# flxrcz/hommx

Hardware: AMD Instinct MI355X
Metric: micro-cell solves/sec (higher is better)
Workload: dtype f64

## Files before the change

### hommx_amd/csrc/fused2d.hip

```cpp
#include <hip/hip_runtime.h>
#include <stdint.h>

#include <type_traits>

#include "kernels.h"
#include "sweep_acc.h"

#ifndef HOMMX_FUSED_WAVES_PER_SIMD
#define HOMMX_FUSED_WAVES_PER_SIMD 2
#endif

namespace hommx {

typedef double d4 __attribute__((ext_vector_type(4)));
typedef double d2 __attribute__((ext_vector_type(2)));

__device__ __forceinline__ double uniform_f64(double v) {
  return __hiloint2double(__builtin_amdgcn_readfirstlane(__double2hiint(v)),
                          __builtin_amdgcn_readfirstlane(__double2loint(v)));
}

struct CoefRow {
  double a0, a1;
  double a0m, a1m;
};

constexpr int MATP = 48;

template <int NB>
struct alignas(16) Lds {
  double mat[(NB + 1) * MATP];
  double ubuf[4 * NB];
  double tsc[16 * 17];
  double rrow[2][NB];
  double vrow[2][NB];
  double vnat[2][NB];
  double e0row[NB];
  double e1row[NB];
  double e0nat[NB];
  double e1nat[NB];
  double dgnat[NB];
  double cenat[NB + 2];
};
template <int NB>
struct alignas(16) LdsIso {
  static constexpr int PARK = NB == 32 ? 12 * 64 : 0;
  double ubuf[4 * NB];
  double tsc[16 * 17];
  double rrow[2][NB];
  double vrow[2][NB];
  double vnat[2][NB];
  double e0row[NB];
  double e0nat[NB];
  double dgnat[NB];
  double cenat[NB + 2];
  double park[PARK ? PARK : 1];
};

struct NoFact {};
template <int NB, bool FACT, bool ISO>
__global__ __launch_bounds__(64, (NB == 32 && ISO) ? 3 : HOMMX_FUSED_WAVES_PER_SIMD) void k_poisson2d_fused(
    const double* __restrict__ coef, const double* __restrict__ Mmat, double* __restrict__ out,
    int32_t* __restrict__ info, int n, long long ncells, const CoefSource src, std::conditional_t<FACT, double*, NoFact> fact
#ifdef HOMMX_FUSED_DEBUG
    , double* __restrict__ dbg
#endif
) {
  constexpr int NT = NB / 16, KK = NB / 4, CG = 64 / NB;
  constexpr int P = MATP;
  constexpr bool PARK = ISO && NB == 32;
  static_assert(!(FACT && ISO), "the factor record keeps the general path");
  __shared__ std::conditional_t<ISO, LdsIso<NB>, Lds<NB>> L;

  const long long cell = blockIdx.x;
  if (cell >= ncells) return;
  __builtin_assume(n >= 3);
  __builtin_assume(n <= NB);
  const int l = threadIdx.x;
  const int j = l & 15, k = l >> 4;
  const int c = l % NB, g = l / NB;
  const int lb = l - c;
  const int p0 = NB - n;
  const bool valid = c >= p0;
  const int cn = c - p0;
  const int cm = valid ? (c == p0 ? NB - 1 : c - 1) : c;
  const int cp = valid ? (c == NB - 1 ? p0 : c + 1) : c;
  const int prow = (c & 3) * KK + (c >> 2);

  const int ownB = (k + 1) * P + j;
  [[maybe_unused]] int leftB[NT];
#pragma unroll
  for (int tj = 0; tj < NT; ++tj) {
    const int col = 16 * tj + j;
    leftB[tj] = (k + 1) * P + (col == p0 ? NB - 1 : col - 1);
  }
#define OWN(ti, tj, r) (ownB + (16 * (ti) + 4 * (r)) * P + 16 * (tj))
#define LEFT(ti, tj, r) (leftB[tj] + (16 * (ti) + 4 * (r)) * P)
  [[maybe_unused]] unsigned matOff = 0;
  if constexpr (!ISO) matOff = accl::lds_offset(&L.mat[0]);
  [[maybe_unused]] const unsigned haloA = matOff + 8u * (unsigned)(p0 * P + j);

  const int mode = src.mode;
  const unsigned char* mask = static_cast<const unsigned char*>(src.table);
  const double* table = static_cast<const double*>(src.table);
  const double* cc = mode == COEF_STREAM ? coef + cell * (2ll * n * n) : coef + cell * 2;
  constexpr int NL = NB * NB / 64;
  double2 pv[NL];
  if (mode == COEF_STREAM) {
#pragma unroll
    for (int i = 0; i < NL; ++i) {
      const int el = 2 * l + 128 * i;
      pv[i] = el < 2 * n * n ? *reinterpret_cast<const double2*>(cc + el) : double2{0.0, 0.0};
    }
  }

  if constexpr (!ISO)
    for (int i = l; i < (NB + 1) * P; i += 64) L.mat[i] = 0.0;
  if (l == 0) L.cenat[0] = 0.0;

  double m00 = 1.0, m01 = 0.0, m10 = 0.0, m11 = 1.0;
  if (!ISO && Mmat) {
    const double* mp = Mmat + cell * 4;
    m00 = mp[0]; m01 = mp[1]; m10 = mp[2]; m11 = mp[3];
  }
  const double al = ISO ? 0.5 : uniform_f64(0.5 * (m00 * m00 + m10 * m10));
  const double be = ISO ? 0.5 : uniform_f64(0.5 * (m01 * m01 + m11 * m11));
  const double ga = ISO ? 0.0 : uniform_f64(0.5 * (m00 * m01 + m10 * m11));
  const double ab = ISO ? 1.0 : uniform_f64(al - 2.0 * ga + be);

  double ph0 = 0.0, ph1 = 0.0;
  if (mode != COEF_STREAM) {
    ph0 = cc[0];
    ph1 = cc[1];
  }
  const int nq = src.nq;
  auto sample = [&](long long el) {
    double acc = 0.0;
    for (int q = 0; q < nq; ++q)
      acc = add_rn(acc, mul_rn(src.weights[q], div_rn(1.0, add_rn(ph0, mul_rn(ph1, table[el * nq + q])))));
    return acc;
  };
  auto load_pair = [&](long long el, double& a0, double& a1) {
    if (mode == COEF_TWO_PHASE) {
      const uchar2 mk = *reinterpret_cast<const uchar2*>(mask + el);
      a0 = mk.x ? ph1 : ph0;
      a1 = mk.y ? ph1 : ph0;
    } else if (mode == COEF_AFFINE) {
      const double2 g2 = *reinterpret_cast<const double2*>(table + el);
      a0 = add_rn(ph0, mul_rn(ph1, g2.x));
      a1 = add_rn(ph0, mul_rn(ph1, g2.y));
    } else if (mode == COEF_RECIPROCAL) {
      a0 = sample(el);
      a1 = sample(el + 1);
    } else {
      const double2 v = *reinterpret_cast<const double2*>(cc + el);
      a0 = v.x; a1 = v.y;
    }
  };
  int esh;
  {
    int ef = 0;
    if (mode == COEF_STREAM) {
      int hm = 0;
#pragma unroll
      for (int i = 0; i < NL; ++i) hm = max(hm, max(__double2hiint(pv[i].x) & 0x7fffffff, __double2hiint(pv[i].y) & 0x7fffffff));
      ef = hm >> 20;
    } else {
      for (long long el = 2 * l; el < 2ll * n * n; el += 128) {
        double a0, a1;
        load_pair(el, a0, a1);
        const int f0 = (__double2hiint(a0) >> 20) & 0x7ff, f1 = (__double2hiint(a1) >> 20) & 0x7ff;
        ef = max(ef, max(f0, f1));
      }
    }
#pragma unroll
    for (int off = 32; off >= 1; off >>= 1) ef = max(ef, __shfl_xor(ef, off, 64));
    const int fm = (__double2hiint(6.0 * (al + be)) >> 20) & 0x7ff;
    const int sh = (ef == 0 || ef == 0x7ff ? 0 : ef - 1023) + (fm == 0 || fm == 0x7ff ? 0 : fm - 1023) + 2;
    esh = __builtin_amdgcn_readfirstlane(ef == 0 || ef == 0x7ff ? 0 : sh);
  }
  auto load_row = [&](int jc) {
    CoefRow r;
    r.a0 = 0.0; r.a1 = 0.0;
    if (valid) {
      load_pair(2 * (jc * n + cn), r.a0, r.a1);
      r.a0 = ldexp(r.a0, -esh);
      r.a1 = ldexp(r.a1, -esh);
    }
    r.a0m = __shfl(r.a0, lb + cm, 64);
    r.a1m = __shfl(r.a1, lb + cm, 64);
    return r;
  };
  auto st_diag = [&](const CoefRow& cur, const CoefRow& prev) {
    return valid ? cur.a0 * al + cur.a1 * be + cur.a0m * ab + prev.a0m * be + prev.a1m * al + prev.a1 * ab : 1.0;
  };
  auto st_E = [&](const CoefRow& cur, const CoefRow& prev) { return (cur.a0 + prev.a1) * (ga - al); };
  auto st_N = [&](const CoefRow& cur) { return (cur.a1 + cur.a0m) * (ga - be); };
  auto st_NE = [&](const CoefRow& cur) { return -ga * (cur.a0 + cur.a1); };
  auto st_p0 = [&](const CoefRow& cur, const CoefRow& prev) { return cur.a0 - cur.a0m - prev.a1m + prev.a1; };
  auto st_p1 = [&](const CoefRow& cur, const CoefRow& prev) { return cur.a1 + cur.a0m - prev.a0m - prev.a1; };

  [[maybe_unused]] auto band_write = [&](double dv, double ov, bool sym, bool clear) {
    if constexpr (!ISO) {
      if (g == 0) {
        const double d_ = clear ? 0.0 : dv, o_ = clear ? 0.0 : ov;
        L.mat[(c + 1) * P + c] = d_;
        if (valid) {
          L.mat[(cp + 1) * P + c] = o_;
          if (sym) L.mat[(c + 1) * P + cp] = o_;
        }
      }
    }
  };
  auto sub_band = [&](double (&x)[NT][NT][4], const double (&dgq)[NT], const double (&ceq)[NT], const double (&cemq)[NT]) {
#pragma unroll
    for (int t = 0; t < NT; ++t) {
      using namespace accl;
#define DIAG_LO(r) (OneLane<0, 4 * (r)>::lo | OneLane<1, 4 * (r) + 1>::lo | OneLane<2, 4 * (r) + 2>::lo | OneLane<3, 4 * (r) + 3>::lo)
#define DIAG_HI(r) (OneLane<0, 4 * (r)>::hi | OneLane<1, 4 * (r) + 1>::hi | OneLane<2, 4 * (r) + 2>::hi | OneLane<3, 4 * (r) + 3>::hi)
      masked_sub4<DIAG_LO(0), DIAG_HI(0), DIAG_LO(1), DIAG_HI(1), DIAG_LO(2), DIAG_HI(2), DIAG_LO(3), DIAG_HI(3)>(
          x[t][t][0], x[t][t][1], x[t][t][2], x[t][t][3], dgq[t]);
#define SUB_LO(r) (((r) ? OneLane<0, (4 * (r) - 1) & 15>::lo : 0u) | OneLane<1, 4 * (r)>::lo | OneLane<2, 4 * (r) + 1>::lo | OneLane<3, 4 * (r) + 2>::lo)
#define SUB_HI(r) (((r) ? OneLane<0, (4 * (r) - 1) & 15>::hi : 0u) | OneLane<1, 4 * (r)>::hi | OneLane<2, 4 * (r) + 1>::hi | OneLane<3, 4 * (r) + 2>::hi)
      masked_sub4<SUB_LO(0), SUB_HI(0), SUB_LO(1), SUB_HI(1), SUB_LO(2), SUB_HI(2), SUB_LO(3), SUB_HI(3)>(
          x[t][t][0], x[t][t][1], x[t][t][2], x[t][t][3], ceq[t]);
#define SUP_LO(r) (OneLane<0, 4 * (r) + 1>::lo | OneLane<1, 4 * (r) + 2>::lo | OneLane<2, 4 * (r) + 3>::lo | ((r) < 3 ? OneLane<3, (4 * (r) + 4) & 15>::lo : 0u))
#define SUP_HI(r) (OneLane<0, 4 * (r) + 1>::hi | OneLane<1, 4 * (r) + 2>::hi | OneLane<2, 4 * (r) + 3>::hi | ((r) < 3 ? OneLane<3, (4 * (r) + 4) & 15>::hi : 0u))
      masked_sub4<SUP_LO(0), SUP_HI(0), SUP_LO(1), SUP_HI(1), SUP_LO(2), SUP_HI(2), SUP_LO(3), SUP_HI(3)>(
          x[t][t][0], x[t][t][1], x[t][t][2], x[t][t][3], cemq[t]);
#undef DIAG_LO
#undef DIAG_HI
#undef SUB_LO
#undef SUB_HI
#undef SUP_LO
#undef SUP_HI
    }
    if (NT == 2) {
      using namespace accl;
      masked_sub<OneLane<0, 15>::lo, OneLane<0, 15>::hi>(x[NT - 1][0][0], ceq[0]);
      masked_sub<OneLane<3, 0>::lo, OneLane<3, 0>::hi>(x[0][NT - 1][3], cemq[NT - 1]);
    }
  };
  [[maybe_unused]] auto band_regs = [&](double (&x)[NT][NT][4], double dv, double ov) {
    double dq[NT], oq[NT], omq[NT];
#pragma unroll
    for (int tj = 0; tj < NT; ++tj) {
      const int col = 16 * tj + j;
      dq[tj] = __shfl(dv, col, 64);
      oq[tj] = __shfl(ov, col, 64);
      const double om = __shfl(ov, (col + 63) & 63, 64);
      omq[tj] = col == 0 ? 0.0 : om;
    }
#pragma unroll
    for (int ti = 0; ti < NT; ++ti)
#pragma unroll
      for (int tj = 0; tj < NT; ++tj)
#pragma unroll
        for (int r = 0; r < 4; ++r) x[ti][tj][r] = 0.0;
    sub_band(x, dq, oq, omq);
    const double cw = readlane_f64(ov, NB - 1);
#pragma unroll
    for (int tj = 0; tj < NT; ++tj) x[NT - 1][tj][3] = (k == 3 && 16 * tj + j == p0) ? x[NT - 1][tj][3] - cw : x[NT - 1][tj][3];
#pragma unroll
    for (int ti = 0; ti < NT; ++ti)
#pragma unroll
      for (int r = 0; r < 4; ++r) x[ti][NT - 1][r] = (j == 15 && 16 * ti + 4 * r + k == p0) ? x[ti][NT - 1][r] - cw : x[ti][NT - 1][r];
  };

  [[maybe_unused]] double* rec = nullptr;
  if constexpr (FACT) rec = fact + cell * fused_fact_doubles(n);
  [[maybe_unused]] double* srec = nullptr;
  if constexpr (FACT) srec = rec + fused_fact_header(NB);

  double wf[NT][KK];
  double a[NT][NT][4];
  d4 slr[NT][NT];
  double rr[2];
  double rlm;
  CoefRow cur;
  double asum;
  __syncthreads();
  {
    const CoefRow rowA = load_row(n - 2);
    const CoefRow rowB = load_row(n - 1);
    cur = load_row(0);
    asum = (rowB.a0 + rowB.a1) + (cur.a0 + cur.a1);
    if constexpr (FACT) {
      const double neB = st_NE(rowB);
      const double c1 = __shfl(neB, lb + cm, 64);
      if (g == 0) {
        rec[c] = st_N(rowB);
        rec[NB + c] = c1;
      }
      if (l < 4) rec[4 * NB + l] = l == 0 ? m00 : l == 1 ? m01 : l == 2 ? m10 : m11;
      if (l == 4) rec[4 * NB + 4] = (double)esh;
    }
    if constexpr (ISO) {
      band_regs(a, -st_diag(rowB, rowA), -st_E(rowB, rowA));
#pragma unroll
      for (int ti = 0; ti < NT; ++ti)
#pragma unroll
        for (int tj = 0; tj <= ti; ++tj)
#pragma unroll
          for (int r = 0; r < 4; ++r) slr[ti][tj][r] = a[ti][tj][r];
      if constexpr (PARK) {
#pragma unroll
        for (int ti = 0; ti < NT; ++ti)
#pragma unroll
          for (int tj = 0; tj <= ti; ++tj)
#pragma unroll
            for (int r = 0; r < 4; ++r) L.park[(4 * (ti * (ti + 1) / 2 + tj) + r) * 64 + l] = slr[ti][tj][r];
      }
      band_regs(a, st_diag(cur, rowB), st_E(cur, rowB));
      const double dv = st_N(rowB);
#pragma unroll
      for (int t = 0; t < NT; ++t) {
        using namespace accl;
#pragma unroll
        for (int kk = 0; kk < KK; ++kk) wf[t][kk] = 0.0;
        const double dq = __shfl(dv, 16 * t + j, 64);
        amov<DiagMask<0>::lo, DiagMask<0>::hi>(wf[t][4 * t], dq);
        amov<DiagMask<1>::lo, DiagMask<1>::hi>(wf[t][4 * t + 1], dq);
        amov<DiagMask<2>::lo, DiagMask<2>::hi>(wf[t][4 * t + 2], dq);
        amov<DiagMask<3>::lo, DiagMask<3>::hi>(wf[t][4 * t + 3], dq);
      }
    } else {
    {
      const double dv = st_diag(rowB, rowA), ov = st_E(rowB, rowA);
      band_write(dv, ov, true, false);
      __syncthreads();
#pragma unroll
      for (int ti = 0; ti < NT; ++ti)
#pragma unroll
        for (int tj = 0; tj <= ti; ++tj)
#pragma unroll
          for (int r = 0; r < 4; ++r) slr[ti][tj][r] = L.mat[OWN(ti, tj, r)];
      __syncthreads();
      band_write(dv, ov, true, true);
      __syncthreads();
    }
    {
      const double dv = st_N(rowB), ov = st_NE(rowB);
      band_write(dv, ov, false, false);
      __syncthreads();
#pragma unroll
      for (int t = 0; t < NT; ++t)
#pragma unroll
        for (int kk = 0; kk < KK; ++kk) wf[t][kk] = L.mat[OWN(kk >> 2, t, kk & 3)];
      __syncthreads();
      band_write(dv, ov, false, true);
      __syncthreads();
    }
    {
      const double dv = -st_diag(cur, rowB), ov = -st_E(cur, rowB);
      band_write(dv, ov, true, false);
      __syncthreads();
#pragma unroll
      for (int ti = 0; ti < NT; ++ti)
#pragma unroll
        for (int tj = 0; tj < NT; ++tj)
#pragma unroll
          for (int r = 0; r < 4; ++r) a[ti][tj][r] = L.mat[OWN(ti, tj, r)];
      __syncthreads();
      band_write(dv, ov, true, true);
      __syncthreads();
    }
    }
    rr[0] = st_p0(cur, rowB); rr[1] = st_p1(cur, rowB);
    rlm = (k >> 1) ? st_p1(rowB, rowA) : st_p0(rowB, rowA);
  }
  double ga_ = 0.0, gb_ = 0.0;
  int bad = 0, badstep = 0;
  [[maybe_unused]] double wselR[NT];
#pragma unroll
  for (int tj = 0; tj < NT; ++tj) wselR[tj] = (k == 3 && 16 * tj + j == p0) ? 1.0 : 0.0;
  [[maybe_unused]] const double wselC = (j == 15 && k == (p0 & 3)) ? 1.0 : 0.0;
  [[maybe_unused]] const int laneR = 48 + (p0 & 15), tileR = p0 >> 4, laneC = 16 * (p0 & 3) + 15;
  double indw[KK];
#pragma unroll
  for (int q = 0; q < KK; ++q) indw[q] = uniform_f64((q == (p0 >> 2)) ? 1.0 : 0.0);

  for (int jr = 0; jr <= n - 2; ++jr) {
    const bool lastStep = (jr == n - 2);
    CoefRow nxt = cur;
    if (!lastStep) {
      nxt = load_row(jr + 1);
      asum += nxt.a0 + nxt.a1;
    }
    const double e0c = st_N(cur);
    [[maybe_unused]] double neC = 0.0, e1c = 0.0;
    if constexpr (!ISO) {
      neC = st_NE(cur);
      e1c = __shfl(neC, lb + cm, 64);
    }
    if (lastStep) {
      if constexpr (ISO) {
#pragma unroll
        for (int t = 0; t < NT; ++t) {
          using namespace accl;
          const double me = -__shfl(e0c, 16 * t + j, 64);
          masked_sub4<DiagMask<0>::lo, DiagMask<0>::hi, DiagMask<1>::lo, DiagMask<1>::hi, DiagMask<2>::lo, DiagMask<2>::hi, DiagMask<3>::lo,
                      DiagMask<3>::hi>(wf[t][4 * t], wf[t][4 * t + 1], wf[t][4 * t + 2], wf[t][4 * t + 3], me);
        }
      } else {
        for (int i = l; i < (NB + 1) * P; i += 64) L.mat[i] = 0.0;
        __syncthreads();
        if (g == 0) {
          L.mat[(c + 1) * P + c] = e0c;
          if (valid) L.mat[(c + 1) * P + cp] = neC;
        }
        __syncthreads();
#pragma unroll
        for (int t = 0; t < NT; ++t)
#pragma unroll
          for (int kk = 0; kk < KK; ++kk) wf[t][kk] += L.mat[OWN(kk >> 2, t, kk & 3)];
        __syncthreads();
      }
    }
    [[maybe_unused]] double pn0 = 0.0, pn1 = 0.0;
    if constexpr (ISO) {
      pn0 = st_p0(nxt, cur);
      pn1 = st_p1(nxt, cur);
    }
    const double dgc = st_diag(nxt, cur), cec = st_E(nxt, cur);
    if (g == 0) {
      L.rrow[0][prow] = rr[0];
      L.rrow[1][prow] = rr[1];
      L.e0row[prow] = e0c;
      if constexpr (!ISO) L.e1row[prow] = e1c;
      L.e0nat[c] = e0c;
      if constexpr (!ISO) L.e1nat[c] = e1c;
      L.dgnat[c] = dgc;
      L.cenat[1 + c] = cec;
    }

    {
      int badj = 0;
#ifdef HOMMX_FUSED_SWEEP32
      accl::Sweep<NB>::run(a, L.ubuf, j, k, badj);
#else
      __builtin_amdgcn_s_setprio(1);
      if constexpr (NB == 32) accl::block_inverse32(a, L.ubuf, L.tsc, j, k, badj);
      else accl::Sweep<NB>::run(a, L.ubuf, j, k, badj);
      __builtin_amdgcn_s_setprio(0);
#endif
      if (badj && !bad) { bad = 1; badstep = jr + 1; }
    }
    if constexpr (FACT) {
#pragma unroll
      for (int ti = 0; ti < NT; ++ti)
#pragma unroll
        for (int tj = 0; tj < NT; ++tj)
#pragma unroll
          for (int r = 0; r < 4; ++r) srec[((ti * NT + tj) * 4 + r) * 64 + l] = a[ti][tj][r];
      if (g == 0) {
        srec[NB * NB + 2 * NB + c] = e0c;
        srec[NB * NB + 3 * NB + c] = e1c;
      }
    }
#ifdef HOMMX_FUSED_DEBUG
    if (dbg && cell == 0) {
      double* q = dbg + (size_t)jr * 4 * NB * NB;
#pragma unroll
      for (int ti = 0; ti < NT; ++ti)
#pragma unroll
        for (int tj = 0; tj < NT; ++tj)
#pragma unroll
          for (int r = 0; r < 4; ++r) q[(16 * ti + 4 * r + k) * NB + 16 * tj + j] = a[ti][tj][r];
#pragma unroll
      for (int t = 0; t < NT; ++t)
#pragma unroll
        for (int kk = 0; kk < KK; ++kk) q[NB * NB + (16 * t + j) * NB + 4 * kk + k] = wf[t][kk];
    }
#endif

    if constexpr (!ISO) if (!lastStep) {
#pragma unroll
      for (int ti = 0; ti < NT; ++ti)
#pragma unroll
        for (int tj = 0; tj < NT; ++tj)
#pragma unroll
          for (int r = 0; r < 4; ++r) L.mat[OWN(ti, tj, r)] = a[ti][tj][r];
#pragma unroll
      for (int tj = 0; tj < NT; ++tj)
        accl::masked_lds_store<accl::RowMask<3>::lo, accl::RowMask<3>::hi>(haloA + 128u * tj, a[NT - 1][tj][3]);
    }

    d4 vt[NT][NT];
#pragma unroll
    for (int x = 0; x < NT; ++x)
#pragma unroll
      for (int y = 0; y < NT; ++y) vt[x][y] = d4{0.0, 0.0, 0.0, 0.0};
#pragma unroll
    for (int kk = 0; kk < KK; ++kk)
#pragma unroll
      for (int x = 0; x < NT; ++x)
#pragma unroll
        for (int y = 0; y < NT; ++y)
          vt[x][y] = __builtin_amdgcn_mfma_f64_16x16x4f64(a[kk >> 2][x][kk & 3], wf[y][kk], vt[x][y], 0, 0, 0);

    if constexpr (PARK) {
#pragma unroll
      for (int x = 0; x < NT; ++x)
#pragma unroll
        for (int y = 0; y <= x; ++y) {
          double* pk = &L.park[4 * (x * (x + 1) / 2 + y) * 64 + l];
          d4 s;
#pragma unroll
          for (int r = 0; r < 4; ++r) s[r] = pk[64 * r];
#pragma unroll
          for (int kk = 0; kk < KK; ++kk) s = __builtin_amdgcn_mfma_f64_16x16x4f64(vt[kk >> 2][x][kk & 3], wf[y][kk], s, 0, 0, 0);
#pragma unroll
          for (int r = 0; r < 4; ++r) pk[64 * r] = s[r];
        }
    } else {
#pragma unroll
    for (int kk = 0; kk < KK; ++kk)
#pragma unroll
      for (int x = 0; x < NT; ++x)
#pragma unroll
        for (int y = 0; y <= x; ++y)
          slr[x][y] = __builtin_amdgcn_mfma_f64_16x16x4f64(vt[kk >> 2][x][kk & 3], wf[y][kk], slr[x][y], 0, 0, 0);
    }

    double z;
    {
      double part[2][NT];
#pragma unroll
      for (int m = 0; m < 2; ++m)
#pragma unroll
        for (int tj = 0; tj < NT; ++tj) part[m][tj] = 0.0;
#pragma unroll
      for (int m = 0; m < 2; ++m)
#pragma unroll
        for (int ti = 0; ti < NT; ++ti) {
          const d4 q = *reinterpret_cast<const d4*>(&L.rrow[m][k * KK + 4 * ti]);
#pragma unroll
          for (int r = 0; r < 4; ++r)
#pragma unroll
            for (int tj = 0; tj < NT; ++tj) part[m][tj] = fma(q[r], a[ti][tj][r], part[m][tj]);
        }
      if (NT == 2) {
        double s_[2];
#pragma unroll
        for (int m = 0; m < 2; ++m) {
          double x = part[m][0], y = part[m][NT - 1];
          swap16(x, y);
          s_[m] = x + y;
        }
        swap32(s_[0], s_[1]);
        z = s_[0] + s_[1];
      } else {
        double x = part[0][0], y = part[1][0];
        swap32(x, y);
        z = add_xor16(x + y);
      }
    }
    if constexpr (ISO) {
      ga_ = fma(z, L.rrow[0][prow], ga_);
      gb_ = fma(z, L.rrow[1][prow], gb_);
    } else {
      ga_ = fma(z, rr[0], ga_);
      gb_ = fma(z, rr[1], gb_);
    }
    L.vnat[k >> 1][c] = z;
    L.vrow[k >> 1][prow] = z;
    if constexpr (FACT) {
      if (NB == 32 || !(k & 1)) srec[NB * NB + (k >> 1) * NB + c] = z;
      srec += fused_fact_step(NB);
    }

    {
      double part[2][NT];
#pragma unroll
      for (int m = 0; m < 2; ++m) {
        double v[KK];
#pragma unroll
        for (int q4 = 0; q4 < KK; q4 += 4) {
          const d4 q = *reinterpret_cast<const d4*>(&L.vrow[m][k * KK + q4]);
          v[q4] = q[0]; v[q4 + 1] = q[1]; v[q4 + 2] = q[2]; v[q4 + 3] = q[3];
        }
#pragma unroll
        for (int t = 0; t < NT; ++t) {
          double acc = 0.0;
#pragma unroll
          for (int kk = 0; kk < KK; ++kk) acc = fma(v[kk], wf[t][kk], acc);
          part[m][t] = acc;
        }
      }
      double z6;
      if (NT == 2) {
        double s_[2];
#pragma unroll
        for (int m = 0; m < 2; ++m) {
          double x = part[m][0], y = part[m][NT - 1];
          swap16(x, y);
          s_[m] = x + y;
        }
        swap32(s_[0], s_[1]);
        z6 = s_[0] + s_[1];
      } else {
        double x = part[0][0], y = part[1][0];
        swap32(x, y);
        z6 = add_xor16(x + y);
      }
      rlm += z6;
    }

    if (!lastStep) {
      [[maybe_unused]] double e0r[KK];
      [[maybe_unused]] double e1r[KK];
#pragma unroll
      for (int q4 = 0; q4 < KK; q4 += 4) {
        if constexpr (!ISO) {
          const d4 x = *reinterpret_cast<const d4*>(&L.e0row[k * KK + q4]);
          const d4 y = *reinterpret_cast<const d4*>(&L.e1row[k * KK + q4]);
          e0r[q4] = x[0]; e0r[q4 + 1] = x[1]; e0r[q4 + 2] = x[2]; e0r[q4 + 3] = x[3];
          e1r[q4] = y[0]; e1r[q4 + 1] = y[1]; e1r[q4 + 2] = y[2]; e1r[q4 + 3] = y[3];
        }
      }
      {
        double e0q[NT], dgq[NT], ceq[NT], cemq[NT];
        [[maybe_unused]] double e1q[NT];
#pragma unroll
        for (int tj = 0; tj < NT; ++tj) {
          e0q[tj] = L.e0nat[16 * tj + j];
          if constexpr (!ISO) e1q[tj] = L.e1nat[16 * tj + j];
          dgq[tj] = L.dgnat[16 * tj + j];
          ceq[tj] = L.cenat[1 + 16 * tj + j];
          cemq[tj] = L.cenat[16 * tj + j];
        }
#pragma unroll
        for (int ti = 0; ti < NT; ++ti)
#pragma unroll
          for (int r = 0; r < 4; ++r)
#pragma unroll
            for (int tj = 0; tj < NT; ++tj) {
              if constexpr (ISO) {
                a[ti][tj][r] = -(L.e0row[k * KK + 4 * ti + r] * (e0q[tj] * a[ti][tj][r]));
              } else {
                const double nl = L.mat[LEFT(ti, tj, r)];
                const double nu = L.mat[OWN(ti, tj, r) - P];
                const double nul = L.mat[LEFT(ti, tj, r) - P];
                const double x = fma(e1q[tj], nl, e0q[tj] * a[ti][tj][r]);
                const double xu = fma(e1q[tj], nul, e0q[tj] * nu);
                a[ti][tj][r] = -fma(e0r[4 * ti + r], x, e1r[4 * ti + r] * xu);
              }
            }
        sub_band(a, dgq, ceq, cemq);
        {
          const double cw = readlane_f64(cec, NB - 1);
#pragma unroll
          for (int tj = 0; tj < NT; ++tj) {
            if constexpr (ISO) a[NT - 1][tj][3] = (l == laneR && tj == tileR) ? fma(-cw, 1.0, a[NT - 1][tj][3]) : fma(-cw, 0.0, a[NT - 1][tj][3]);
            else a[NT - 1][tj][3] = fma(-cw, wselR[tj], a[NT - 1][tj][3]);
          }
          double vcol;
          if constexpr (ISO) vcol = l == laneC ? -cw : -cw * 0.0;
          else vcol = -cw * wselC;
#pragma unroll
          for (int ti = 0; ti < NT; ++ti)
#pragma unroll
            for (int r = 0; r < 4; ++r) a[ti][NT - 1][r] = fma(vcol, indw[4 * ti + r], a[ti][NT - 1][r]);
        }
      }

      if constexpr (ISO) {
#pragma unroll
        for (int kk = 0; kk < KK; ++kk)
#pragma unroll
          for (int t = 0; t < NT; ++t) wf[t][kk] = L.e0row[k * KK + kk] * vt[kk >> 2][t][kk & 3];
      } else {
#pragma unroll
        for (int x = 0; x < NT; ++x)
#pragma unroll
          for (int y = 0; y < NT; ++y)
#pragma unroll
            for (int r = 0; r < 4; ++r) L.mat[OWN(x, y, r)] = vt[x][y][r];
#pragma unroll
        for (int y = 0; y < NT; ++y)
          accl::masked_lds_store<accl::RowMask<3>::lo, accl::RowMask<3>::hi>(haloA + 128u * y, vt[NT - 1][y][3]);
#pragma unroll
        for (int t = 0; t < NT; ++t)
#pragma unroll
          for (int kk = 0; kk < KK; ++kk) {
            const double up = L.mat[OWN(kk >> 2, t, kk & 3) - P];
            wf[t][kk] = fma(e1r[kk], up, e0r[kk] * vt[kk >> 2][t][kk & 3]);
          }
      }

      {
        const double v0 = L.vnat[0][c], v1 = L.vnat[1][c];
        if constexpr (ISO) {
          const double e0 = L.e0nat[c];
          rr[0] = fma(v0, e0, pn0);
          rr[1] = fma(v1, e0, pn1);
        } else {
          const double vm0 = L.vnat[0][cm], vm1 = L.vnat[1][cm];
          rr[0] = fma(vm0, e1c, fma(v0, e0c, st_p0(nxt, cur)));
          rr[1] = fma(vm1, e1c, fma(v1, e0c, st_p1(nxt, cur)));
        }
      }
      cur = nxt;
      __syncthreads();
    }
  }

  int lt = l, jt = j, kt = k, ct = c, prowt = prow;
  if constexpr (ISO) {
    lt = (int)__lane_id();
    asm volatile("" : "+v"(lt));
    jt = lt & 15;
    kt = lt >> 4;
    ct = lt % NB;
    prowt = (ct & 3) * KK + (ct >> 2);
  }
  {
  const int l = lt, j = jt, k = kt, c = ct, prow = prowt;
  [[maybe_unused]] auto bfly = [&](double v, int off) {
    const int ad = (l ^ off) << 2;
    return __hiloint2double(__builtin_amdgcn_ds_bpermute(ad, __double2hiint(v)), __builtin_amdgcn_ds_bpermute(ad, __double2loint(v)));
  };
  {
    if constexpr (PARK) {
#pragma unroll
      for (int ti = 0; ti < NT; ++ti)
#pragma unroll
        for (int tj = 0; tj <= ti; ++tj)
#pragma unroll
          for (int r = 0; r < 4; ++r) slr[ti][tj][r] = L.park[(4 * (ti * (ti + 1) / 2 + tj) + r) * 64 + l];
    }
    [[maybe_unused]] d4 sup = d4{0.0, 0.0, 0.0, 0.0};
    if (NT == 2) {
      if constexpr (ISO) {
        sup = accl::transpose_tile(slr[NT - 1][0], L.tsc, j, k);
      } else {
#pragma unroll
        for (int r = 0; r < 4; ++r) L.mat[OWN(1, 0, r)] = slr[NT - 1][0][r];
        __syncthreads();
      }
    }
#pragma unroll
    for (int ti = 0; ti < NT; ++ti)
#pragma unroll
      for (int tj = 0; tj < NT; ++tj)
#pragma unroll
        for (int r = 0; r < 4; ++r) {
          if (tj <= ti) a[ti][tj][r] = -slr[ti][tj][r];
          else if constexpr (ISO) a[ti][tj][r] = -sup[r];
          else a[ti][tj][r] = -L.mat[(16 + j + 1) * P + 4 * r + k];
        }
    {
      using namespace accl;
#pragma unroll
      for (int tj = 0; tj < NT; ++tj) amov<RowMask<3>::lo, RowMask<3>::hi>(a[NT - 1][tj][3], 0.0);
#pragma unroll
      for (int ti = 0; ti < NT; ++ti)
#pragma unroll
        for (int r = 0; r < 4; ++r) amov<ColMask<15>::lo, ColMask<15>::hi>(a[ti][NT - 1][r], 0.0);
      amov<OneLane<3, 15>::lo, OneLane<3, 15>::hi>(a[NT - 1][NT - 1][3], -1.0);
    }
    if (c == NB - 1) rlm = 0.0;
    __syncthreads();
    L.rrow[k >> 1][prow] = rlm;
    L.vnat[k >> 1][c] = rlm;
    __syncthreads();
    int badj = 0;
    accl::Sweep<NB>::run(a, L.ubuf, j, k, badj);
    if (badj && !bad) { bad = 1; badstep = n; }
    if constexpr (FACT) {
#pragma unroll
      for (int ti = 0; ti < NT; ++ti)
#pragma unroll
        for (int tj = 0; tj < NT; ++tj)
#pragma unroll
          for (int r = 0; r < 4; ++r) srec[((ti * NT + tj) * 4 + r) * 64 + l] = a[ti][tj][r];
    }
    double part[2][NT];
#pragma unroll
    for (int m = 0; m < 2; ++m)
#pragma unroll
      for (int tj = 0; tj < NT; ++tj) part[m][tj] = 0.0;
#pragma unroll
    for (int m = 0; m < 2; ++m)
#pragma unroll
      for (int ti = 0; ti < NT; ++ti) {
        const d4 q = *reinterpret_cast<const d4*>(&L.rrow[m][k * KK + 4 * ti]);
#pragma unroll
        for (int r = 0; r < 4; ++r)
#pragma unroll
          for (int tj = 0; tj < NT; ++tj) part[m][tj] = fma(q[r], a[ti][tj][r], part[m][tj]);
      }
    double z;
    if (NT == 2) {
      double s_[2];
#pragma unroll
      for (int m = 0; m < 2; ++m) {
        double x = part[m][0], y = part[m][NT - 1];
        swap16(x, y);
        s_[m] = x + y;
      }
      swap32(s_[0], s_[1]);
      z = s_[0] + s_[1];
    } else {
      double x = part[0][0], y = part[1][0];
      swap32(x, y);
      z = add_xor16(x + y);
    }
    ga_ = fma(z, L.vnat[0][c], ga_);
    gb_ = fma(z, L.vnat[1][c], gb_);
    if constexpr (FACT) {
      if (NB == 32 || !(k & 1)) rec[2 * NB + (k >> 1) * NB + c] = z;
    }
  }

  double g00 = (k < 2) ? ga_ : 0.0, g01 = (k < 2) ? gb_ : 0.0, g11 = (k < 2) ? 0.0 : gb_;
#pragma unroll
  for (int off = 32; off >= 1; off >>= 1) {
    if constexpr (ISO) {
      g00 += bfly(g00, off);
      g01 += bfly(g01, off);
      g11 += bfly(g11, off);
      asum += bfly(asum, off);
    } else {
      g00 += __shfl_xor(g00, off, 64);
      g01 += __shfl_xor(g01, off, 64);
      g11 += __shfl_xor(g11, off, 64);
      asum += __shfl_xor(asum, off, 64);
    }
  }
  if (l == 0) {
    const double h = 1.0 / n;
    constexpr int DUP = 32 / NB;
    const double sc = 0.25 * h * h / DUP;
    const double c0 = 0.5 * h * h * asum / CG;
    const double t00 = m00 * g00 + m01 * g01, t01 = m00 * g01 + m01 * g11;
    const double t10 = m10 * g00 + m11 * g01, t11 = m10 * g01 + m11 * g11;
    double* o = out + cell * 4;
    o[0] = ldexp(c0 + sc * (t00 * m00 + t01 * m01), esh);
    o[1] = ldexp(sc * (t00 * m10 + t01 * m11), esh);
    o[2] = ldexp(sc * (t10 * m00 + t11 * m01), esh);
    o[3] = ldexp(c0 + sc * (t10 * m10 + t11 * m11), esh);
    if (info) info[cell] = bad ? badstep : 0;
  }
  }
#undef OWN
#undef LEFT
}

#ifndef HOMMX_DEV_LDS_PAD
#define HOMMX_DEV_LDS_PAD 0
#endif
#ifdef HOMMX_FUSED_DEBUG
extern double* g_fused_dbg;
#define HOMMX_FUSED_LDS 0
#define HOMMX_FUSED_DBG_ARG , g_fused_dbg
#else
#define HOMMX_FUSED_LDS HOMMX_DEV_LDS_PAD
#define HOMMX_FUSED_DBG_ARG
#endif

#if defined(HOMMX_FUSED_ISO_TU)
hipError_t launch_poisson2d_fused_iso(const double* d_coef, double* d_out, int32_t* d_info, int n, long long ncells, hipStream_t stream,
                                      CoefSource src) {
  if (ncells <= 0) return hipSuccess;
  dim3 grid((unsigned)ncells), block(64);
  const double* d_M = nullptr;
  if (n <= 16)
    hipLaunchKernelGGL((k_poisson2d_fused<16, false, true>), grid, block, HOMMX_FUSED_LDS, stream, d_coef, d_M, d_out, d_info, n, ncells, src,
                       NoFact{} HOMMX_FUSED_DBG_ARG);
  else
    hipLaunchKernelGGL((k_poisson2d_fused<32, false, true>), grid, block, HOMMX_FUSED_LDS, stream, d_coef, d_M, d_out, d_info, n, ncells, src,
                       NoFact{} HOMMX_FUSED_DBG_ARG);
  return hipGetLastError();
}

#elif !defined(HOMMX_FUSED_FACT_TU)
hipError_t launch_poisson2d_fused(const double* d_coef, const double* d_M, double* d_out, int32_t* d_info,
                                  int n, long long ncells, hipStream_t stream, CoefSource src) {
  if (ncells <= 0) return hipSuccess;
  if (!d_M) return launch_poisson2d_fused_iso(d_coef, d_out, d_info, n, ncells, stream, src);
  dim3 grid((unsigned)ncells), block(64);
  if (n <= 16)
    hipLaunchKernelGGL((k_poisson2d_fused<16, false, false>), grid, block, HOMMX_FUSED_LDS, stream, d_coef, d_M, d_out, d_info, n, ncells, src,
                       NoFact{} HOMMX_FUSED_DBG_ARG);
  else
    hipLaunchKernelGGL((k_poisson2d_fused<32, false, false>), grid, block, HOMMX_FUSED_LDS, stream, d_coef, d_M, d_out, d_info, n, ncells, src,
                       NoFact{} HOMMX_FUSED_DBG_ARG);
  return hipGetLastError();
}

#else
hipError_t launch_poisson2d_fused_fact(const double* d_coef, const double* d_M, double* d_out, int32_t* d_info, int n, long long ncells,
                                       hipStream_t stream, double* d_fact) {
  if (ncells <= 0) return hipSuccess;
  dim3 grid((unsigned)ncells), block(64);
  const CoefSource src;
  if (n <= 16)
    hipLaunchKernelGGL((k_poisson2d_fused<16, true, false>), grid, block, 0, stream, d_coef, d_M, d_out, d_info, n, ncells, src,
                       d_fact HOMMX_FUSED_DBG_ARG);
  else
    hipLaunchKernelGGL((k_poisson2d_fused<32, true, false>), grid, block, 0, stream, d_coef, d_M, d_out, d_info, n, ncells, src,
                       d_fact HOMMX_FUSED_DBG_ARG);
  return hipGetLastError();
}
#endif

}
```

Before: 8.702 million.

## Exploit diagonal first-step weights and skip padded k-slabs in isotropic MFMA sweep

For the isotropic path, the first sweep step (jr==0) has a diagonal weight matrix. Its update is therefore computed with elementwise FMAs scaled by the diagonal read from LDS, replacing two chains of MFMA products. On later steps, when the cell is padded (p0>0), k-slabs that lie entirely in the padding are skipped in both MFMA chains. This adds branches, extra LDS writes of the diagonal, and a tile transpose, and the results depend on the padded entries being zero.

```diff
diff --git a/hommx_amd/csrc/fused2d.hip b/hommx_amd/csrc/fused2d.hip
--- a/hommx_amd/csrc/fused2d.hip
+++ b/hommx_amd/csrc/fused2d.hip
@@ -69,6 +69,11 @@
   constexpr int NT = NB / 16, KK = NB / 4, CG = 64 / NB;
   constexpr int P = MATP;
   constexpr bool PARK = ISO && NB == 32;
+#ifdef HOMMX_FUSED_SWEEP32
+  constexpr bool ZSLAB = false;
+#else
+  constexpr bool ZSLAB = ISO;
+#endif
   static_assert(!(FACT && ISO), "the factor record keeps the general path");
   __shared__ std::conditional_t<ISO, LdsIso<NB>, Lds<NB>> L;
 
@@ -81,6 +86,7 @@
   const int c = l % NB, g = l / NB;
   const int lb = l - c;
   const int p0 = NB - n;
+  [[maybe_unused]] const int kk0 = p0 >> 2;
   const bool valid = c >= p0;
   const int cn = c - p0;
   const int cm = valid ? (c == p0 ? NB - 1 : c - 1) : c;
@@ -324,6 +330,10 @@
         amov<DiagMask<2>::lo, DiagMask<2>::hi>(wf[t][4 * t + 2], dq);
         amov<DiagMask<3>::lo, DiagMask<3>::hi>(wf[t][4 * t + 3], dq);
       }
+      if (g == 0) {
+        L.vnat[0][c] = dv;
+        L.vrow[0][prow] = dv;
+      }
     } else {
     {
       const double dv = st_diag(rowB, rowA), ov = st_E(rowB, rowA);
@@ -487,6 +497,82 @@
     }
 
     d4 vt[NT][NT];
+    if (ZSLAB && jr == 0) {
+      if constexpr (ZSLAB) {
+        int l0 = (int)__lane_id();
+        asm volatile("" : "+v"(l0));
+        const int j0 = l0 & 15, k0 = l0 >> 4;
+        double dcol[NT];
+#pragma unroll
+        for (int t = 0; t < NT; ++t) dcol[t] = L.vnat[0][16 * t + j0];
+#pragma unroll
+        for (int x = 0; x < NT; ++x) {
+          const d4 dr = *reinterpret_cast<const d4*>(&L.vrow[0][k0 * KK + 4 * x]);
+#pragma unroll
+          for (int y = 0; y <= x; ++y) {
+            if constexpr (PARK) {
+              double* pk = &L.park[4 * (x * (x + 1) / 2 + y) * 64 + l0];
+#pragma unroll
+              for (int r = 0; r < 4; ++r) pk[64 * r] = fma(fma(a[x][y][r], dr[r], 0.0), dcol[y], pk[64 * r]);
+            } else {
+#pragma unroll
+              for (int r = 0; r < 4; ++r) slr[x][y][r] = fma(fma(a[x][y][r], dr[r], 0.0), dcol[y], slr[x][y][r]);
+            }
+          }
+        }
+#pragma unroll
+        for (int x = 0; x < NT; ++x)
+#pragma unroll
+          for (int y = 0; y < NT; ++y) {
+            d4 nt = d4{a[x][y][0], a[x][y][1], a[x][y][2], a[x][y][3]};
+            if (x == y) nt = accl::transpose_tile(nt, L.tsc, j0, k0);
+#pragma unroll
+            for (int r = 0; r < 4; ++r) vt[x][y][r] = fma(nt[r], dcol[y], 0.0);
+          }
+      }
+    } else if (ZSLAB && kk0 != 0) {
+      if constexpr (ZSLAB) {
+#pragma unroll
+        for (int x = 0; x < NT; ++x)
+#pragma unroll
+          for (int y = 0; y < NT; ++y) vt[x][y] = d4{0.0, 0.0, 0.0, 0.0};
+#pragma unroll
+        for (int kk = 0; kk < KK; ++kk)
+          if (kk >= 3 || kk >= kk0) {
+#pragma unroll
+            for (int x = 0; x < NT; ++x)
+#pragma unroll
+              for (int y = 0; y < NT; ++y)
+                vt[x][y] = __builtin_amdgcn_mfma_f64_16x16x4f64(a[kk >> 2][x][kk & 3], wf[y][kk], vt[x][y], 0, 0, 0);
+          }
+        if constexpr (PARK) {
+#pragma unroll
+          for (int x = 0; x < NT; ++x)
+#pragma unroll
+            for (int y = 0; y <= x; ++y) {
+              double* pk = &L.park[4 * (x * (x + 1) / 2 + y) * 64 + l];
+              d4 s;
+#pragma unroll
+              for (int r = 0; r < 4; ++r) s[r] = pk[64 * r];
+#pragma unroll
+              for (int kk = 0; kk < KK; ++kk)
+                if (kk >= 3 || kk >= kk0) s = __builtin_amdgcn_mfma_f64_16x16x4f64(vt[kk >> 2][x][kk & 3], wf[y][kk], s, 0, 0, 0);
+#pragma unroll
+              for (int r = 0; r < 4; ++r) pk[64 * r] = s[r];
+            }
+        } else {
+#pragma unroll
+          for (int kk = 0; kk < KK; ++kk)
+            if (kk >= 3 || kk >= kk0) {
+#pragma unroll
+              for (int x = 0; x < NT; ++x)
+#pragma unroll
+                for (int y = 0; y <= x; ++y)
+                  slr[x][y] = __builtin_amdgcn_mfma_f64_16x16x4f64(vt[kk >> 2][x][kk & 3], wf[y][kk], slr[x][y], 0, 0, 0);
+            }
+        }
+      }
+    } else {
 #pragma unroll
     for (int x = 0; x < NT; ++x)
 #pragma unroll
@@ -521,6 +607,7 @@
 #pragma unroll
         for (int y = 0; y <= x; ++y)
           slr[x][y] = __builtin_amdgcn_mfma_f64_16x16x4f64(vt[kk >> 2][x][kk & 3], wf[y][kk], slr[x][y], 0, 0, 0);
+    }
     }
 
     double z;
```

Result: no change. 8.767 million, median of 6 (+0.8%).
